# Enigmatisms/cuda-pt

Measured on AMD Instinct MI355X. Metric: Msamples/sec (whole node), 1080p modern-kitchen, higher is better.
Workload: dtype fp32; 1 GPU; model=modern-kitchen-proc, global_batch=32, seq_len=2073600, width=1920, height=1080, renderer=pt, n_prims=131444, parallelism=dp1 (sample-split, RCCL all-reduce)

## Files before the change

csrc/bind.cpp:

```cpp
#include <pybind11/pybind11.h>
#include <pybind11/numpy.h>
#include <pybind11/stl.h>
#include <algorithm>
#include <cstring>
#include <stdexcept>

#include "core/scene_view.h"
#include "core/integrator.h"
#include "cpu/bvh_build.h"
#include "hip/kernels.h"
#include "hip/lds_plan.h"

namespace py = pybind11;
using namespace hippt;

namespace hippt {
void render_cpu(const SceneView& sv, float* accum, float* var,
                int spp0, int nspp, uint32_t seed, int renderer, int n_threads,
                int y0, int y1, const uint8_t* spp_map, float* aux);
void render_lt_cpu(const SceneView& sv, float* accum, int spp0, int nspp, uint32_t seed,
                   int spec_constraint, float caustic_scaling, int n_threads);
}

namespace {

using farr = py::array_t<float, py::array::c_style | py::array::forcecast>;
using iarr = py::array_t<int32_t, py::array::c_style | py::array::forcecast>;
using uarr = py::array_t<uint32_t, py::array::c_style | py::array::forcecast>;

#define HIP_OK(expr)                                                                   \
    do {                                                                               \
        int _e = (expr);                                                               \
        if (_e != 0) throw std::runtime_error(std::string("HIP error ") +              \
                                              std::to_string(_e) + " at " #expr);      \
    } while (0)

Vec3 to_vec3(const std::vector<float>& v) { return {v[0], v[1], v[2]}; }

int super_cell_voxels() {
    static const int SUP = [] {
        const char* e = getenv("HIPPT_SUPER_N");
        int v = e ? atoi(e) : 16;
        return v < 2 ? 2 : (v > 64 ? 64 : v);
    }();
    return SUP;
}

inline void super_splat(std::vector<float>& sup, const MediumParams& m, int SUP,
                        int ix, int iy, int iz, float v) {
    int cx0 = std::max(0, (ix - 1) / SUP), cx1 = std::min(m.sx - 1, (ix + 1) / SUP);
    int cy0 = std::max(0, (iy - 1) / SUP), cy1 = std::min(m.sy - 1, (iy + 1) / SUP);
    int cz0 = std::max(0, (iz - 1) / SUP), cz1 = std::min(m.sz - 1, (iz + 1) / SUP);
    for (int cz = cz0; cz <= cz1; ++cz)
        for (int cy = cy0; cy <= cy1; ++cy)
            for (int cx = cx0; cx <= cx1; ++cx) {
                float& s = sup[(size_t(cz) * m.sy + cy) * m.sx + cx];
                s = fmaxf(s, v);
            }
}

int bvh4_tree_depth(const BVH4Node* nodes, int n) {
    if (n <= 0) return 0;
    std::vector<std::pair<int, int>> stk{{0, 1}};
    int maxd = 1;
    while (!stk.empty()) {
        auto [idx, d] = stk.back();
        stk.pop_back();
        maxd = std::max(maxd, d);
        const BVH4Node& nd = nodes[idx];
        for (int c = 0; c < 4; ++c)
            if (nd.child[c] >= 0 && !(nd.child[c] == 0 && nd.cnt[c] == 0))
                stk.push_back({nd.child[c], d + 1});
    }
    return maxd;
}

static std::vector<uint64_t> host_lds_slots(int lds_n);

std::vector<uint32_t> make_prim_shade(const uint32_t* prim_obj, size_t n_prims,
                                      const int32_t* objs, size_t n_objs) {
    std::vector<uint32_t> out(n_prims);
    int bad = -1;
    if (!build_prim_shade(prim_obj, (int)n_prims, objs, (int)n_objs, out.data(), &bad))
        throw std::runtime_error(
            "build_prim_shade: primitive " + std::to_string(bad) +
            " needs object < n_objs, 0 <= bsdf_id < " + std::to_string(SHADE_MAX_BSDFS) +
            " and emitter_id < " + std::to_string(SHADE_MAX_EMITTERS));
    return out;
}

struct SceneHolder {
    farr np_prims, np_attrs, np_nodes, np_nodes4, np_nodes8;
    uarr np_prim_obj;
    iarr np_objs;
    std::vector<BsdfParams> bsdfs;
    std::vector<EmitterParams> emitters;
    std::vector<PhaseParams> phases;
    std::vector<MediumParams> media;
    std::vector<farr> media_density, media_temp;
    std::vector<std::vector<float>> media_super;
    std::vector<std::vector<int32_t>> media_bricks;
    std::vector<int> media_nbricks;
    std::vector<farr> tex_data;
    std::vector<TexView> tex_host;
    std::vector<int> emitter_prims;
    std::vector<float> emitter_cdf;
    std::vector<uint32_t> prim_shade;
    std::vector<LightPrim> light_prims;
    bool shade_stale = true;
    std::vector<float> env_rows_h, env_cols_h;
    int env_w = 0, env_h = 0;
    std::vector<float> emitter_sel_h;
    Camera cam{};
    MaxDepthParams md{};
    int env_emitter = -1;
    int cam_medium = -1;

    bool has_dev = false;
    int device_id = 0;
    std::vector<void*> dev_bufs;
    std::vector<TexView> tex_dev;
    std::vector<MediumParams> media_dev;
    void* dev_bsdfs = nullptr;
    void* dev_emitters = nullptr;
    void* dev_media = nullptr;

    SceneView host_sv{};
    SceneView dev_sv{};
    WfState* wf = nullptr;

    ~SceneHolder() { release(); }

    void release() {
        if (wf) { wf_destroy(wf); wf = nullptr; }
        for (void* p : dev_bufs) dev_free(p);
        dev_bufs.clear();
        has_dev = false;
    }

    void set_geometry(farr prims, farr attrs, uarr prim_obj, farr nodes, farr nodes4,
                      farr nodes8) {
        if (prims.ndim() != 2 || prims.shape(1) != 12) throw std::runtime_error("prims must be (n,12)");
        if (attrs.ndim() != 2 || attrs.shape(1) != 16) throw std::runtime_error("attrs must be (n,16)");
        if (nodes.ndim() != 2 || nodes.shape(1) != 8) throw std::runtime_error("nodes must be (m,8)");
        if (nodes4.ndim() == 2 && nodes4.shape(0) > 0 && nodes4.shape(1) != 32)
            throw std::runtime_error("nodes4 must be (m,32)");
        np_prims = std::move(prims);
        np_attrs = std::move(attrs);
        np_prim_obj = std::move(prim_obj);
        shade_stale = true;
        np_nodes = std::move(nodes);
        np_nodes4 = std::move(nodes4);
        if (nodes8.ndim() == 2 && nodes8.shape(0) > 0 && nodes8.shape(1) != 64)
            throw std::runtime_error("nodes8 must be (m,64)");
        np_nodes8 = std::move(nodes8);
        bvh4_depth = np_nodes4.ndim() == 2 && np_nodes4.shape(0) > 0
            ? bvh4_tree_depth((const BVH4Node*)np_nodes4.data(), (int)np_nodes4.shape(0))
            : 0;
        nodes4q = np_nodes4.ndim() == 2 && np_nodes4.shape(0) > 0
            ? quantize_bvh4((const BVH4Node*)np_nodes4.data(), (int)np_nodes4.shape(0))
            : std::vector<BVH4NodeQ>();
        nodes4t = np_nodes4.ndim() == 2 && np_nodes4.shape(0) > 0
            ? tag_bvh4((const BVH4Node*)np_nodes4.data(), (int)np_nodes4.shape(0))
            : std::vector<BVH4NodeT>();
        const Prim* pr = (const Prim*)np_prims.data();
        const uint32_t* po = np_prim_obj.data();
        int n = (int)np_prims.shape(0);
        AABB sb;
        for (int i = 0; i < n; ++i) {
            if (po[i] & PRIM_SPHERE_BIT) {
                Vec3 c = pr[i].v0.xyz();
                float rad = pr[i].v0.w;
                sb.grow(c - Vec3(rad)); sb.grow(c + Vec3(rad));
            } else {
                Vec3 v0 = pr[i].v0.xyz();
                sb.grow(v0);
                sb.grow(v0 + pr[i].e1.xyz());
                sb.grow(v0 + pr[i].e2.xyz());
            }
        }
        Vec3 c = (sb.lo + sb.hi) * 0.5f;
        float rad = n > 0 ? (sb.hi - sb.lo).length() * 0.5f : 1.f;
        scene_bound = Vec4(c, rad);
        tri_only = 1;
        for (int i = 0; i < n; ++i)
            if (po[i] & PRIM_SPHERE_BIT) { tri_only = 0; break; }
    }

    int bvh4_depth = 0;
    Vec4 scene_bound{0.f, 0.f, 0.f, 1.f};
    int cache_nodes = 0;
    int tri_only = 0;
    std::vector<BVH4NodeQ> nodes4q;
    std::vector<BVH4NodeT> nodes4t;

    void set_cache_level(int level) {
        cache_nodes = level > 0 ? (1 << (level > 12 ? 12 : level)) : 0;
    }

    void set_objects(iarr objs) {
        if (objs.ndim() != 2 || objs.shape(1) != 8) throw std::runtime_error("objs must be (n,8)");
        np_objs = std::move(objs);
        shade_stale = true;
    }

    int add_bsdf(int type, std::vector<float> kd, std::vector<float> ks, std::vector<float> kg,
                 float ior, float extra0, float extra1, std::vector<int> tex) {
        BsdfParams b = BsdfParams::make(type);
        b.kd = Vec4(kd[0], kd[1], kd[2], kd.size() > 3 ? kd[3] : 0.f);
        b.ks = Vec4(ks[0], ks[1], ks[2], ks.size() > 3 ? ks[3] : 0.f);
        b.kg = Vec4(kg[0], kg[1], kg[2], kg.size() > 3 ? kg[3] : 0.f);
        b.ior = ior; b.extra0 = extra0; b.extra1 = extra1;
        for (size_t i = 0; i < tex.size() && i < 8; ++i) b.tex[i] = (int16_t)tex[i];
        bsdfs.push_back(b);
        return (int)bsdfs.size() - 1;
    }

// ... 722 lines not shown
            }
            if (wk0.rec.prim_idx < 0) wk0.rec.t = MAX_DIST;
            if (wk1.rec.prim_idx < 0) wk1.rec.t = MAX_DIST;
            if (!same_hit(b, wk0.rec) || !same_hit(b, wk1.rec)) { ++bad; continue; }
        }
        if (n8p) {
            HitRecord w8 = ray_intersect_bvh8_ww(n8p, pr, po, r, tmax, lds, lds_n);
            bool occ8 = occlusion_test_bvh8(n8p, pr, po, r, tmax, lds, lds_n);
            bool occ_ref = occlusion_test_bvh4(n4, pr, po, r, tmax, lds, lds_n);
            if (!same_hit(b, w8) || occ8 != occ_ref) { ++bad; continue; }
        }
        bool occ_a = occlusion_test_bvh(bn, n_nodes, pr, po, r, tmax);
        bool occ_b = occlusion_test_bvh4(n4, pr, po, r, tmax, lds, lds_n);
        if (occlusion_test_bvh4_ww(t4, pr, po, r, tmax, lds, lds_n) != occ_b) { ++bad; continue; }
        if (!same_hit(a, b) || occ_a != occ_b) ++bad;
    }
    return bad;
}

int py_bvh4q_selftest(farr prims, uarr prim_obj, farr nodes4,
                      farr ray_o, farr ray_d, float tmax, int lds_n) {
    const BVH4Node* n4 = (const BVH4Node*)nodes4.data();
    int nn = (int)nodes4.shape(0);
    std::vector<BVH4NodeQ> q = quantize_bvh4(n4, nn);
    const std::vector<BVH4NodeT> t4v = tag_bvh4(n4, nn);
    const BVH4NodeT* t4 = t4v.data();
    const Prim* pr = (const Prim*)prims.data();
    const uint32_t* po = prim_obj.data();
    std::vector<uint64_t> slots = host_lds_slots(lds_n);
    LdsSlot lds = bvh_host_slot(lds_n ? slots.data() : nullptr);
    int bad = 0;
    int nr = (int)ray_o.shape(0);
    for (int i = 0; i < nr; ++i) {
        Ray r;
        r.o = {ray_o.at(i, 0), ray_o.at(i, 1), ray_o.at(i, 2)};
        r.d = {ray_d.at(i, 0), ray_d.at(i, 1), ray_d.at(i, 2)};
        HitRecord a = ray_intersect_bvh4_ww(t4, pr, po, r, tmax, lds, lds_n);
        HitRecord b = ray_intersect_bvh4q_ww(q.data(), pr, po, r, tmax, lds, lds_n);
        if (!same_hit(a, b)) { ++bad; continue; }
        bool oa = occlusion_test_bvh4_ww(t4, pr, po, r, tmax, lds, lds_n);
        bool ob = occlusion_test_bvh4q_ww(q.data(), pr, po, r, tmax, lds, lds_n);
        if (oa != ob) ++bad;
    }
    return bad;
}

uarr py_bvh4_tag(farr nodes4) {
    if (nodes4.ndim() != 2 || nodes4.shape(1) != 32) throw std::runtime_error("nodes4 must be (m,32)");
    const std::vector<BVH4NodeT> t4 =
        tag_bvh4((const BVH4Node*)nodes4.data(), (int)nodes4.shape(0));
    uarr out({(py::ssize_t)t4.size(), (py::ssize_t)32});
    std::memcpy(out.mutable_data(), t4.data(), t4.size() * sizeof(BVH4NodeT));
    return out;
}

int py_bvh4_visit_selftest(farr nodes4, farr ray_o, farr ray_d, float tmax) {
    if (nodes4.ndim() != 2 || nodes4.shape(1) != 32) throw std::runtime_error("nodes4 must be (m,32)");
    const BVH4Node* n4 = (const BVH4Node*)nodes4.data();
    const int nn = (int)nodes4.shape(0);
    const std::vector<BVH4NodeT> t4 = tag_bvh4(n4, nn);
    const LdsSlot no_lds = nullptr;
    int bad = 0;
    const int nr = (int)ray_o.shape(0);
    for (int i = 0; i < nr; ++i) {
        Ray r;
        r.o = {ray_o.at(i, 0), ray_o.at(i, 1), ray_o.at(i, 2)};
        r.d = {ray_d.at(i, 0), ray_d.at(i, 1), ray_d.at(i, 2)};
        const Vec3 inv_d = safe_rcp_dir(r.d);
        const Vec3 o_div = r.o * inv_d;
        for (int j = 0; j < nn; ++j) {
            uint64_t sa[4] = {0, 0, 0, 0}, sb[4] = {0, 0, 0, 0};
            int spa = 0, spb = 0;
            uint32_t na, nb;
            {
                const BVH4Node nd = n4[j];
                BVH_VISIT_ORDERED(BVH4Node, na, nd, inv_d, o_div, tmax, sa, spa, no_lds, 0)
            }
            {
                const BVH4NodeT nd = t4[j];
                BVH_VISIT_TAGGED4(nb, nd, inv_d, o_div, tmax, sb, spb, no_lds, 0)
            }
            if (na != nb || spa != spb || std::memcmp(sa, sb, sizeof(sa)) != 0) ++bad;
        }
    }
    return bad;
}

int py_bvh4_any_visit_selftest(farr nodes4, farr ray_o, farr ray_d, float tmax) {
    if (nodes4.ndim() != 2 || nodes4.shape(1) != 32) throw std::runtime_error("nodes4 must be (m,32)");
    const BVH4Node* n4 = (const BVH4Node*)nodes4.data();
    const int nn = (int)nodes4.shape(0);
    const std::vector<BVH4NodeT> t4 = tag_bvh4(n4, nn);
    const LdsSlot no_lds = nullptr;
    auto collect = [](uint32_t next, const uint64_t* st, int sp, uint32_t* out, int& n) {
        n = 0;
        if (next != BVH4_NONE_W) out[n++] = next;
        for (int k = 0; k < sp; ++k) {
            if (st[k] >> 32) return false;
            const uint32_t w = (uint32_t)st[k];
            if (w == BVH4_NONE_W || w == BVH4_ANY_MISS_W) return false;
            out[n++] = w;
        }
        std::sort(out, out + n);
        return std::adjacent_find(out, out + n) == out + n;
    };
    int bad = 0;
// ... 114 lines not shown
        .def("add_bsdf", &SceneHolder::add_bsdf)
        .def("update_bsdf", &SceneHolder::update_bsdf)
        .def("add_emitter", &SceneHolder::add_emitter)
        .def("update_emitter", &SceneHolder::update_emitter)
        .def("set_emitter_prims", &SceneHolder::set_emitter_prims)
        .def("set_env_cdf", &SceneHolder::set_env_cdf)
        .def("set_emitter_sel", &SceneHolder::set_emitter_sel)
        .def("add_phase", &SceneHolder::add_phase)
        .def("add_medium", &SceneHolder::add_medium)
        .def("add_medium_sparse", &SceneHolder::add_medium_sparse)
        .def("media_info", &SceneHolder::media_info)
        .def("medium_super", &SceneHolder::medium_super)
        .def("update_medium", &SceneHolder::update_medium)
        .def("add_texture", &SceneHolder::add_texture)
        .def("set_camera", &SceneHolder::set_camera)
        .def("set_depths", &SceneHolder::set_depths,
             py::arg("max_depth"), py::arg("max_diffuse"), py::arg("max_specular"),
             py::arg("max_transmit"), py::arg("max_volume"), py::arg("min_time"),
             py::arg("max_time"), py::arg("use_tof"), py::arg("radiance_clamp") = 0.f)
        .def("set_cache_level", &SceneHolder::set_cache_level)
        .def_readwrite("cam_medium", &SceneHolder::cam_medium)
        .def_readwrite("env_emitter", &SceneHolder::env_emitter)
        .def("finalize", &SceneHolder::finalize)
        .def("upload", &SceneHolder::upload)
        .def("release", &SceneHolder::release)
        .def("render_host", &SceneHolder::render_host,
             py::arg("accum"), py::arg("var"), py::arg("spp0"), py::arg("nspp"),
             py::arg("seed"), py::arg("renderer"), py::arg("spec_constraint"),
             py::arg("caustic_scaling"), py::arg("n_threads"),
             py::arg("y0") = 0, py::arg("y1") = 0, py::arg("spp_map") = py::none(),
             py::arg("aux") = py::none())
        .def("render_device", &SceneHolder::render_device,
             py::arg("accum_ptr"), py::arg("var_ptr"), py::arg("spp0"), py::arg("nspp"),
             py::arg("seed"), py::arg("renderer"), py::arg("spec_constraint"),
             py::arg("caustic_scaling"), py::arg("stream"),
             py::arg("y0") = 0, py::arg("y1") = 0, py::arg("spp_map_ptr") = 0,
             py::arg("aux_ptr") = 0)
        .def("trace_rays", &SceneHolder::trace_rays, py::arg("o"), py::arg("d"),
             py::arg("tmax"), py::arg("device"), py::arg("lds_n") = -1,
             py::arg("n_cached") = -1)
        .def("shade_probe", &SceneHolder::shade_probe_py, py::arg("prim_idx"),
             py::arg("device"))
        .def("tables", &SceneHolder::tables)
        .def("info", &SceneHolder::info);

    m.def("build_bvh", &py_build_bvh, py::arg("prims"), py::arg("prim_obj"),
          py::arg("max_leaf") = 4, py::arg("overlap_w") = 0.f,
          py::arg("use_sbvh") = false, py::arg("ref_unsplit") = true,
          py::arg("trav_cost") = 0.f);
    m.def("collapse_bvh4", &py_collapse_bvh4, py::arg("nodes"));
    m.def("collapse_bvh8", &py_collapse_bvh8, py::arg("nodes"));
    m.def("bvh4_hit", &py_bvh4_hit);
    m.def("bvh4_tag", &py_bvh4_tag, py::arg("nodes4"));
    m.def("bvh4_visit_selftest", &py_bvh4_visit_selftest, py::arg("nodes4"),
          py::arg("ray_o"), py::arg("ray_d"), py::arg("tmax"));
    m.def("bvh4_any_visit_selftest", &py_bvh4_any_visit_selftest, py::arg("nodes4"),
          py::arg("ray_o"), py::arg("ray_d"), py::arg("tmax"));
    m.def("build_prim_shade", [](uarr prim_obj, iarr objs) {
        if (objs.ndim() != 2 || objs.shape(1) != 8) throw std::runtime_error("objs must be (n,8)");
        std::vector<uint32_t> w = make_prim_shade(prim_obj.data(), (size_t)prim_obj.size(),
                                                  objs.data(), (size_t)objs.shape(0));
        uarr out((py::ssize_t)w.size());
        if (!w.empty()) std::memcpy(out.mutable_data(), w.data(), w.size() * 4);
        return out;
    }, py::arg("prim_obj"), py::arg("objs"));
    m.def("build_light_prims", [](farr prims, farr attrs, uarr prim_obj, iarr emitter_prims) {
        if (prims.ndim() != 2 || prims.shape(1) != 12) throw std::runtime_error("prims must be (n,12)");
        if (attrs.ndim() != 2 || attrs.shape(1) != 16) throw std::runtime_error("attrs must be (n,16)");
        const py::ssize_t n_prims = prims.shape(0);
        if (attrs.shape(0) != n_prims || prim_obj.size() != n_prims)
            throw std::runtime_error("prims, attrs and prim_obj must have one row per primitive");
        const py::ssize_t n = emitter_prims.size();
        for (py::ssize_t k = 0; k < n; ++k)
            if (emitter_prims.data()[k] < 0 || emitter_prims.data()[k] >= n_prims)
                throw std::runtime_error("emitter_prims entry outside the primitive array");
        uarr out({n, (py::ssize_t)32});
        build_light_prims((const Prim*)prims.data(), (const PrimAttr*)attrs.data(),
                          prim_obj.data(), emitter_prims.data(), (size_t)n,
                          (LightPrim*)out.mutable_data());
        return out;
    }, py::arg("prims"), py::arg("attrs"), py::arg("prim_obj"), py::arg("emitter_prims"));
    m.def("bsdf_check", &py_bsdf_check);
    m.def("env_check", &py_env_check);
    m.def("bvh4q_selftest", &py_bvh4q_selftest,
          py::arg("prims"), py::arg("prim_obj"), py::arg("nodes4"),
          py::arg("ray_o"), py::arg("ray_d"), py::arg("tmax"), py::arg("lds_n") = 0);
    m.def("bvh4_selftest", &py_bvh4_selftest,
          py::arg("prims"), py::arg("prim_obj"), py::arg("nodes"), py::arg("nodes4"),
          py::arg("ray_o"), py::arg("ray_d"), py::arg("tmax"),
          py::arg("nodes8") = farr(), py::arg("lds_n") = 0);

    m.def("wf_sort_probe", [](uarr status, uarr gather, int mode) {
        if (status.ndim() != 1 || gather.ndim() != 1)
            throw std::runtime_error("wf_sort_probe: status (n,), gather (m,) or empty");
        const int n = (int)status.shape(0), m = (int)gather.shape(0);
        uarr out(n);
        int live = -1;
        HIP_OK(wf_sort_probe(status.data(), n, gather.data(), m, mode,
                             out.mutable_data(), &live));
        return py::make_tuple(out, live);
    }, py::arg("status"), py::arg("gather"), py::arg("mode"));
    m.def("lds_plan", [](int occ, bool stack_in_lds, bool scratch_drops_cache, int n_nodes4,
                         int node_bytes, int cache_req, int lds_req) {
        if (n_nodes4 < 0 || node_bytes <= 0) throw std::runtime_error("lds_plan: bad sizes");
        const LdsPlan p = lds_plan(occ, stack_in_lds, scratch_drops_cache, n_nodes4,
                                   node_bytes, cache_req, lds_req);
        return py::make_tuple(p.lds_n, p.n_cached, p.shmem);
    }, py::arg("occ"), py::arg("stack_in_lds"), py::arg("scratch_drops_cache"),
       py::arg("n_nodes4"), py::arg("node_bytes"), py::arg("cache_req"),
       py::arg("lds_req") = -1);
    m.def("dev_synchronize", [] { HIP_OK(dev_synchronize()); });
    m.def("dev_set_device", [](int d) { HIP_OK(dev_set_device(d)); });

    m.def("struct_sizes", [] {
        py::dict d;
        d["BVHNode"] = (int)sizeof(BVHNode);
        d["Prim"] = (int)sizeof(Prim);
        d["PrimAttr"] = (int)sizeof(PrimAttr);
        d["ObjInfo"] = (int)sizeof(ObjInfo);
        d["BsdfParams"] = (int)sizeof(BsdfParams);
        d["EmitterParams"] = (int)sizeof(EmitterParams);
        d["MediumParams"] = (int)sizeof(MediumParams);
        d["PhaseParams"] = (int)sizeof(PhaseParams);
        d["TexView"] = (int)sizeof(TexView);
        d["Camera"] = (int)sizeof(Camera);
        d["SceneView"] = (int)sizeof(SceneView);
        return d;
    });

    m.attr("R_MEGAKERNEL_PT") = (int)R_MEGAKERNEL_PT;
    m.attr("R_WAVEFRONT_PT") = (int)R_WAVEFRONT_PT;
    m.attr("R_VOLUME_PT") = (int)R_VOLUME_PT;
    m.attr("R_LIGHT_TRACE") = (int)R_LIGHT_TRACE;
    m.attr("R_DEPTH") = (int)R_DEPTH;
    m.attr("R_BVH_COST") = (int)R_BVH_COST;
    m.attr("R_MEGAKERNEL_PT_DYN") = (int)R_MEGAKERNEL_PT_DYN;
    m.attr("WAVE_SIZE") = 64;
}
```

csrc/core/bvh4.h:

```cpp
#pragma once
#include <stdexcept>
#include "bvh.h"

namespace hippt {

template <int W>
struct alignas(16) BVHWideNode {
    static constexpr int WIDTH = W;
    static constexpr bool EMPTY_BEFORE_BOX = false;
    static constexpr bool TAGGED = false;
    float lo_x[W], lo_y[W], lo_z[W];
    float hi_x[W], hi_y[W], hi_z[W];
    int32_t child[W];
    int32_t cnt[W];
};
using BVH4Node = BVHWideNode<4>;
static_assert(sizeof(BVH4Node) == 128, "BVH4Node must be 128 bytes");

struct alignas(16) BVH4NodeT {
    static constexpr int WIDTH = 4;
    static constexpr bool EMPTY_BEFORE_BOX = false;
    static constexpr bool TAGGED = true;
    float lo_x[4], lo_y[4], lo_z[4];
    float hi_x[4], hi_y[4], hi_z[4];
    uint32_t child[4];
    uint32_t pad[4];
};
static_assert(sizeof(BVH4NodeT) == 128, "BVH4NodeT must be 128 bytes");

struct alignas(16) BVH4NodeQ {
    static constexpr int WIDTH = 4;
    static constexpr bool EMPTY_BEFORE_BOX = true;
    static constexpr bool TAGGED = true;
    float ox, oy, oz;
    uint8_t ex, ey, ez;
    uint8_t pad;
    uint8_t qlo[4][3];
    uint8_t qhi[4][3];
    uint32_t child[4];
};
static_assert(sizeof(BVH4NodeQ) == 64, "BVH4NodeQ must be 64 bytes");

constexpr int BVH4_STACK = 64;

constexpr uint32_t BVH4_NONE_W = 0x7fffffffu;
HD uint32_t bvh4_filled_word(int ch, int pc) {
    return ch < 0 ? (0x80000000u | ((uint32_t)pc << 27) | (uint32_t)(~ch)) : (uint32_t)ch;
}
HD uint32_t bvh4_child_word(int ch, int pc) {
    if (ch < 0 && pc == 0) return BVH4_NONE_W;
    return bvh4_filled_word(ch, pc);
}
HD bool bvh4_is_leaf(uint32_t w) { return w >= 0x80000000u; }
HD bool bvh4_not_leaf(uint32_t w) { return w < 0x80000000u; }
// ... 245 lines not shown
    }
#define BVH_VISIT_ANY4(next, nd, inv_d, o_div, tmax, stack, sp, lds_slot, lds_n) \
    BVH_ANY_WORD4(w0_, nd, 0, inv_d, o_div, tmax)                         \
    BVH_ANY_WORD4(w1_, nd, 1, inv_d, o_div, tmax)                         \
    BVH_ANY_WORD4(w2_, nd, 2, inv_d, o_div, tmax)                         \
    BVH_ANY_WORD4(w3_, nd, 3, inv_d, o_div, tmax)                         \
    BVH_ANY_MINMAX(w0_, w1_)                                              \
    BVH_ANY_MINMAX(w2_, w3_)                                              \
    BVH_ANY_MINMAX(w0_, w2_)                                              \
    BVH_ANY_MINMAX(w1_, w3_)                                              \
    BVH_ANY_MINMAX(w1_, w2_)                                              \
    BVH_PUSH_ANY4(w3_, stack, sp, lds_slot, lds_n)                        \
    BVH_PUSH_ANY4(w2_, stack, sp, lds_slot, lds_n)                        \
    BVH_PUSH_ANY4(w1_, stack, sp, lds_slot, lds_n)                        \
    next = w0_ == BVH4_ANY_MISS_W ? BVH4_NONE_W : w0_;

HD Prim bvh_load_prim(const Prim* prims, const uint32_t* prim_obj, int pid,
                      bool tri_only, bool& sph) {
    uint32_t obj = 0;
    if (!tri_only) obj = prim_obj[pid];
    const Prim p = prims[pid];
#if HIPPT_ON_DEVICE
    asm volatile("" :: "v"(obj), "v"(p.v0.x), "v"(p.v0.y), "v"(p.v0.z), "v"(p.v0.w),
                       "v"(p.e1.x), "v"(p.e1.y), "v"(p.e1.z), "v"(p.e1.w),
                       "v"(p.e2.x), "v"(p.e2.y), "v"(p.e2.z), "v"(p.e2.w));
#endif
    sph = (obj & PRIM_SPHERE_BIT) != 0;
    return p;
}
HD void bvh4_leaf_hit(const Prim* prims, const uint32_t* prim_obj,
                      const Ray& ray, int base, int cnt, HitRecord& rec,
                      bool tri_only = false) {
    for (int k = 0; k < cnt; ++k) {
        int pid = base + k;
        bool sph;
        const Prim p = bvh_load_prim(prims, prim_obj, pid, tri_only, sph);
        float u, v;
        float t = intersect_prim(p, sph, ray, u, v);
        if (t > EPSILON && t < rec.t) {
            rec.t = t; rec.u = u; rec.v = v; rec.prim_idx = pid;
        }
    }
}
#define BVH_LEAF_ANY_RETURN(prims, prim_obj, ray, base, cnt, tmax, tri_only)  \
    for (int k_ = 0; k_ < (cnt); ++k_) {                                      \
        int pid_ = (base) + k_;                                               \
        bool sph_;                                                            \
        const Prim p_ = bvh_load_prim(prims, prim_obj, pid_, tri_only, sph_); \
        float u_, v_;                                                         \
        float t_ = intersect_prim(p_, sph_, ray, u_, v_);                     \
        if (t_ > EPSILON && t_ < (tmax)) return true;                         \
    }

template <class Node>
HD HitRecord bvh_closest_ww(const Node* nodes, const Prim* prims,
                            const uint32_t* prim_obj, const Ray& ray, float tmax,
                            LdsSlot lds_slot, int lds_n, const Node* top_cache,
                            int n_cached, bool tri_only) {
    HitRecord rec;
    rec.t = tmax;
    const Vec3 inv_d = safe_rcp_dir(ray.d);
    const Vec3 o_div = ray.o * inv_d;
    uint64_t stack[BVH4_STACK];
    int sp = 0;
    uint32_t cur = 0;
    for (;;) {
        while (bvh4_is_node(cur)) {
            const Node* nsrc = (int)cur < n_cached ? top_cache : nodes;
            const Node nd = nsrc[cur];
            uint32_t next;
            BVH_VISIT(Node, next, nd, inv_d, o_div, rec.t, stack, sp, lds_slot, lds_n)
            if (next != BVH4_NONE_W) { cur = next; continue; }
            BVH_POP_CLOSER(cur, stack, sp, lds_slot, lds_n, rec.t, break, break)
        }
        if (cur == BVH4_NONE_W) break;
        while (bvh4_is_leaf(cur)) {
            bvh4_leaf_hit(prims, prim_obj, ray, bvh4_leaf_base(cur),
                          bvh4_leaf_count(cur), rec, tri_only);
            BVH_POP_CLOSER(cur, stack, sp, lds_slot, lds_n, rec.t, break, break)
        }
        if (cur == BVH4_NONE_W) break;
    }
    if (rec.prim_idx < 0) rec.t = MAX_DIST;
    return rec;
}
template <class Node>
HD bool bvh_any_ww(const Node* nodes, const Prim* prims, const uint32_t* prim_obj,
                   const Ray& ray, float tmax, LdsSlot lds_slot, int lds_n,
                   const Node* top_cache, int n_cached, bool tri_only) {
    const Vec3 inv_d = safe_rcp_dir(ray.d);
    const Vec3 o_div = ray.o * inv_d;
    uint64_t stack[BVH4_STACK];
    int sp = 0;
    uint32_t cur = 0;
    for (;;) {
        while (bvh4_is_node(cur)) {
            const Node* nsrc = (int)cur < n_cached ? top_cache : nodes;
            const Node nd = nsrc[cur];
            uint32_t next = BVH4_NONE_W;
            if constexpr (BVH4_ANY_STRAIGHT && Node::WIDTH == 4 && Node::TAGGED) {
                BVH_VISIT_ANY4(next, nd, inv_d, o_div, tmax, stack, sp, lds_slot, lds_n)
            } else {
                BVH_VISIT_ANY_EACH(Node, next, nd, inv_d, o_div, tmax, stack, sp, lds_slot, lds_n)
            }
            if (next != BVH4_NONE_W) { cur = next; continue; }
            BVH_POP_WORD(cur, stack, sp, lds_slot, lds_n, break)
        }
        if (cur == BVH4_NONE_W) return false;
        while (bvh4_is_leaf(cur)) {
            const int base = bvh4_leaf_base(cur), pc = bvh4_leaf_count(cur);
            BVH_LEAF_ANY_RETURN(prims, prim_obj, ray, base, pc, tmax, tri_only)
            BVH_POP_WORD(cur, stack, sp, lds_slot, lds_n, break)
        }
        if (cur == BVH4_NONE_W) return false;
    }
}

HD HitRecord ray_intersect_bvh4_ww(const BVH4NodeT* nodes,
                                   const Prim* prims, const uint32_t* prim_obj,
                                   const Ray& ray, float tmax,
                                   LdsSlot lds_slot = nullptr, int lds_n = 0,
                                   const BVH4NodeT* top_cache = nullptr,
                                   int n_cached = 0, bool tri_only = false) {
    return bvh_closest_ww(nodes, prims, prim_obj, ray, tmax, lds_slot, lds_n,
                          top_cache, n_cached, tri_only);
}
HD bool occlusion_test_bvh4_ww(const BVH4NodeT* nodes,
                               const Prim* prims, const uint32_t* prim_obj,
                               const Ray& ray, float tmax,
                               LdsSlot lds_slot = nullptr, int lds_n = 0,
                               const BVH4NodeT* top_cache = nullptr,
                               int n_cached = 0, bool tri_only = false) {
    return bvh_any_ww(nodes, prims, prim_obj, ray, tmax, lds_slot, lds_n,
                      top_cache, n_cached, tri_only);
}
HD HitRecord ray_intersect_bvh4q_ww(const BVH4NodeQ* nodes,
                                    const Prim* prims, const uint32_t* prim_obj,
                                    const Ray& ray, float tmax,
                                    LdsSlot lds_slot = nullptr, int lds_n = 0,
                                    const BVH4NodeQ* top_cache = nullptr,
                                    int n_cached = 0) {
    return bvh_closest_ww(nodes, prims, prim_obj, ray, tmax, lds_slot, lds_n,
                          top_cache, n_cached, false);
}
HD bool occlusion_test_bvh4q_ww(const BVH4NodeQ* nodes,
                                const Prim* prims, const uint32_t* prim_obj,
                                const Ray& ray, float tmax,
                                LdsSlot lds_slot = nullptr, int lds_n = 0,
                                const BVH4NodeQ* top_cache = nullptr,
                                int n_cached = 0) {
    return bvh_any_ww(nodes, prims, prim_obj, ray, tmax, lds_slot, lds_n,
// ... 106 lines not shown
}

struct Bvh4Walk {
    HitRecord rec;
    uint32_t cur;
    int sp;
    Vec3 inv_d, o_div;
    Ray ray;
    uint64_t stack[BVH4_STACK / 2];
};

HD void bvh4_walk_init(Bvh4Walk& w, const Ray& ray, float tmax) {
    w.rec = HitRecord();
    w.rec.t = tmax;
    w.cur = 0;
    w.sp = 0;
    w.inv_d = safe_rcp_dir(ray.d);
    w.o_div = ray.o * w.inv_d;
    w.ray = ray;
}

HD bool bvh4_walk_step(Bvh4Walk& w, const BVH4NodeT* nodes, const Prim* prims,
                       const uint32_t* prim_obj, LdsSlot lds_slot, int lds_n) {
    if (w.cur == BVH4_NONE_W) return false;
    if (bvh4_not_leaf(w.cur)) {
        const BVH4NodeT nd = nodes[w.cur];
        uint32_t next;
        BVH_VISIT_TAGGED4(next, nd, w.inv_d, w.o_div, w.rec.t,
                          w.stack, w.sp, lds_slot, lds_n)
        if (next != BVH4_NONE_W) { w.cur = next; return true; }
    } else {
        bvh4_leaf_hit(prims, prim_obj, w.ray, bvh4_leaf_base(w.cur),
                      bvh4_leaf_count(w.cur), w.rec);
    }
    BVH_POP_CLOSER(w.cur, w.stack, w.sp, lds_slot, lds_n, w.rec.t, return false, return true)
}

inline std::vector<BVH4NodeT> tag_bvh4(const BVH4Node* nodes, int n) {
    std::vector<BVH4NodeT> out((size_t)(n > 0 ? n : 0));
    for (int i = 0; i < n; ++i) {
        const BVH4Node& s = nodes[i];
        BVH4NodeT& t = out[i];
        std::memcpy(t.lo_x, s.lo_x, 6 * 4 * sizeof(float));
        for (int c = 0; c < 4; ++c) {
            if (s.child[c] < 0 && (int64_t)(~s.child[c]) + s.cnt[c] > BVH4_MAX_PRIMS)
                throw std::runtime_error("tag_bvh4: leaf beyond BVH4_MAX_PRIMS prims");
            t.child[c] = bvh4_child_word(s.child[c], s.cnt[c]);
            t.pad[c] = 0;
        }
    }
    return out;
}

inline std::vector<BVH4NodeQ> quantize_bvh4(const BVH4Node* nodes, int n) {
    std::vector<BVH4NodeQ> out((size_t)n);
    for (int i = 0; i < n; ++i) {
        const BVH4Node& s = nodes[i];
        BVH4NodeQ& q = out[i];
        float lo[3] = {3e38f, 3e38f, 3e38f}, hi[3] = {-3e38f, -3e38f, -3e38f};
        for (int c = 0; c < 4; ++c) {
            if (s.child[c] == 0 && s.cnt[c] == 0) continue;
            lo[0] = fminf(lo[0], s.lo_x[c]); hi[0] = fmaxf(hi[0], s.hi_x[c]);
            lo[1] = fminf(lo[1], s.lo_y[c]); hi[1] = fmaxf(hi[1], s.hi_y[c]);
            lo[2] = fminf(lo[2], s.lo_z[c]); hi[2] = fmaxf(hi[2], s.hi_z[c]);
        }
        if (lo[0] > hi[0]) { lo[0] = lo[1] = lo[2] = 0.f; hi[0] = hi[1] = hi[2] = 0.f; }
        q.ox = lo[0]; q.oy = lo[1]; q.oz = lo[2];
        uint8_t* eptr = &q.ex;
        for (int a = 0; a < 3; ++a) {
            float ext = fmaxf(hi[a] - lo[a], 0.f);
            int e = 127;
            if (ext > 0.f) {
                float need = ext / 255.f;
                int ee;
                frexpf(need, &ee);
                e = 127 + ee;
                if (e < 1) e = 1;
                if (e > 254) e = 254;
            }
            eptr[a] = (uint8_t)e;
        }
        q.pad = 0;
        const float sxyz[3] = {bvh4q_scale(q.ex), bvh4q_scale(q.ey), bvh4q_scale(q.ez)};
        for (int c = 0; c < 4; ++c) {
            if (s.child[c] == 0 && s.cnt[c] == 0) {
                q.child[c] = BVH4_NONE_W;
                for (int a = 0; a < 3; ++a) { q.qlo[c][a] = 255; q.qhi[c][a] = 0; }
                continue;
            }
            const float clo[3] = {s.lo_x[c], s.lo_y[c], s.lo_z[c]};
            const float chi[3] = {s.hi_x[c], s.hi_y[c], s.hi_z[c]};
            for (int a = 0; a < 3; ++a) {
                float inv_s = 1.f / sxyz[a];
                float fl = floorf((clo[a] - (&q.ox)[a]) * inv_s);
                float fh = ceilf((chi[a] - (&q.ox)[a]) * inv_s);
                q.qlo[c][a] = (uint8_t)clampv((int)fl, 0, 255);
                q.qhi[c][a] = (uint8_t)clampv((int)fh, 0, 255);
            }
            q.child[c] = bvh4_child_word(s.child[c], s.cnt[c]);
        }
    }
    return out;
}

}
```

csrc/hip/pt_kernels.hip:

```cpp
#include <hip/hip_runtime.h>
#include "kernels.h"
#include "trav_lds.h"
#include <climits>
#include "../core/integrator.h"
#include "../core/integrator_vol.h"
#include "../core/light_tracer.h"

namespace hippt {

__device__ inline int xcd_swizzle(int flat, int n_tiles) {
    int xcd = flat & 7, local = flat >> 3;
    int per = n_tiles >> 3, rem = n_tiles & 7;
    return xcd * per + (xcd < rem ? xcd : rem) + local;
}

template <int RENDERER, int MINW, bool BRICKS = false>
__global__ __launch_bounds__(256)
__attribute__((amdgpu_waves_per_eu(MINW, MINW)))
void k_render(SceneView sv, float* __restrict__ accum, float* __restrict__ var,
              int spp0, int nspp, uint32_t seed, int swiz, int lds_n, int n_cached, int y_off, int y_end,
              const uint8_t* __restrict__ spp_map, float* __restrict__ aux) {
    extern __shared__ uint64_t s_stk[];
    TravCtx tc = trav_lds_ctx(sv, s_stk, threadIdx.y * 16 + threadIdx.x, lds_n, n_cached);
    int tile = blockIdx.y * gridDim.x + blockIdx.x;
// ... 78 lines not shown
            Sampler sp(uint32_t(pix), uint32_t(spp0 + s) * SEED_SCALER + seed);
            Ray ray = sv.cam.gen_ray(px, py, sp, spp0 + s);
            Vec3 L = trace_path(sv, ray, sp, tc);
            Lsum += L;
            float lum = (L.x + L.y + L.z) * (1.f / 3.f);
            lum_s += lum;
            lum_s2 = fmaf(lum, lum, lum_s2);
        }
        float* a = accum + pix * 4;
        a[0] += Lsum.x; a[1] += Lsum.y; a[2] += Lsum.z; a[3] += (float)nspp;
        if (var) { var[pix * 2 + 0] += lum_s; var[pix * 2 + 1] += lum_s2; }
    }
}

__global__ __launch_bounds__(256)
__attribute__((amdgpu_waves_per_eu(6, 6)))
void k_render_lt(SceneView sv, float* __restrict__ accum,
                 long long n_paths, int spp0, int nspp, uint32_t seed,
                 int spec_constraint, float caustic_scaling, int lds_n) {
    extern __shared__ uint64_t s_stk[];
    TravCtx tc{(LdsSlot)&s_stk[threadIdx.x], lds_n};
    const long long stride = (long long)gridDim.x * blockDim.x;
    for (long long i = (long long)blockIdx.x * blockDim.x + threadIdx.x; i < n_paths; i += stride) {
        Sampler sp(uint32_t(i & 0xffffffff), uint32_t(spp0) * SEED_SCALER + seed + uint32_t(i >> 32));
        trace_light_path_impl(sv, sp, [&](int pix, Vec3 v) {
            atomicAdd(accum + pix * 4 + 0, v.x);
            atomicAdd(accum + pix * 4 + 1, v.y);
            atomicAdd(accum + pix * 4 + 2, v.z);
        }, tc, spec_constraint, caustic_scaling);
    }
}

__global__ void k_add_count(float* __restrict__ accum, size_t npix, float cnt) {
    size_t i = (size_t)blockIdx.x * blockDim.x + threadIdx.x;
    if (i < npix) accum[i * 4 + 3] += cnt;
}

int launch_render(const SceneView& sv, float* accum, float* var,
                  int spp0, int nspp, uint32_t seed, int renderer,
                  int spec_constraint, float caustic_scaling, void* stream,
                  int y0, int y1, const uint8_t* spp_map, float* aux) {
    hipStream_t st = (hipStream_t)stream;
    static const int swiz_v = env_int("HIPPT_SWIZZLE", 0);
    const int swiz = renderer == R_DEPTH || renderer == R_BVH_COST ? 0 : swiz_v;
    constexpr int OCC_PT = 4, OCC_VPT = 4, OCC_REST = 4, OCC_UNSET = INT_MIN;
    static const int occ_env = env_int("HIPPT_OCC", OCC_UNSET);
    const bool is_rest = renderer == R_LIGHT_TRACE || renderer == R_DEPTH ||
                         renderer == R_BVH_COST || renderer == R_MEGAKERNEL_PT_DYN;
    const int occ_v = occ_env != OCC_UNSET ? occ_env
                    : renderer == R_VOLUME_PT ? OCC_VPT
                    : is_rest ? OCC_REST : OCC_PT;
    static const bool stack_in_lds = !env_is("HIPPT_STACK", "scratch");
    const LdsPlan plan = lds_plan(occ_v, stack_in_lds, false, sv.n_nodes4,
                                  (int)sizeof(TravNode), top_cache_request(sv));
    const int lds_n = plan.lds_n, n_cached = plan.n_cached;
    const uint32_t shmem = plan.shmem;
    const int w = sv.cam.w, h = sv.cam.h;
    if (y1 <= 0 || y1 > h) y1 = h;
    if (y0 < 0) y0 = 0;
    dim3 block(16, 16);
    dim3 grid((w + 15) / 16, (y1 - y0 + 15) / 16);
    void (*k)(SceneView, float*, float*, int, int, uint32_t, int, int, int, int, int,
              const uint8_t*, float*) = nullptr;
    switch (renderer) {
    case R_LIGHT_TRACE: {
        long long n_paths = (long long)w * h * nspp;
        int nblk = 256 * 8 * 4;
        hipLaunchKernelGGL(k_render_lt, dim3(nblk), dim3(256), shmem, st,
                           sv, accum, n_paths, spp0, nspp, seed, spec_constraint, caustic_scaling, lds_n);
        size_t npix = (size_t)w * h;
        hipLaunchKernelGGL(k_add_count, dim3((npix + 255) / 256), dim3(256), 0, st,
                           accum, npix, (float)nspp);
        break;
    }
    case R_VOLUME_PT:
        if (sv.media_bricks) k = occ_v == 4 ? k_render<R_VOLUME_PT, 4, true> : k_render<R_VOLUME_PT, 6, true>;
        else k = occ_v == 4 ? k_render<R_VOLUME_PT, 4> : k_render<R_VOLUME_PT, 6>;
        break;
    case R_DEPTH: k = k_render<R_DEPTH, 6>; break;
    case R_BVH_COST: k = k_render<R_BVH_COST, 6>; break;
    case R_MEGAKERNEL_PT_DYN: {
        static struct Counters {
            uint32_t* p[64] = {};
            ~Counters() { for (uint32_t* q : p) if (q) (void)hipFree(q); }
        } counters;
        int dev = 0;
        (void)hipGetDevice(&dev);
        uint32_t*& counter = counters.p[dev & 63];
        if (!counter) {
            if (hipMalloc((void**)&counter, 4) != hipSuccess) return (int)hipGetLastError();
        }
        (void)hipMemsetAsync(counter, 0, 4, st);
        int tiles_x = (w + 15) / 16, tiles_y = (h + 15) / 16;
        hipLaunchKernelGGL((k_render_persistent<R_MEGAKERNEL_PT, 6>), dim3(256 * 4), block, shmem, st,
                           sv, accum, var, spp0, nspp, seed, counter, tiles_x,
                           tiles_x * tiles_y, lds_n);
        break;
    }
    default:
        if (occ_v <= 3) k = k_render<R_MEGAKERNEL_PT, 3>;
        else if (occ_v == 4) k = k_render<R_MEGAKERNEL_PT, 4>;
        else if (occ_v == 5) k = k_render<R_MEGAKERNEL_PT, 5>;
        else if (occ_v >= 8) k = k_render<R_MEGAKERNEL_PT, 8>;
        else k = k_render<R_MEGAKERNEL_PT, 6>;
        break;
    }
    if (k) hipLaunchKernelGGL(k, grid, block, shmem, st, sv, accum, var, spp0, nspp, seed,
// ... 17 lines not shown
```

csrc/hip/trav_lds.h:

```cpp
#pragma once
#include <hip/hip_runtime.h>
#include <cstdlib>
#include <cstring>
#include "lds_plan.h"
#include "../core/scene_view.h"

namespace hippt {

inline int env_int(const char* name, int dflt) {
    const char* e = getenv(name);
    return e ? atoi(e) : dflt;
}
inline bool env_is(const char* name, const char* value) {
    const char* e = getenv(name);
    return e && strcmp(e, value) == 0;
}

inline int top_cache_request(const SceneView& sv, int probe = -1) {
    static const int cache_env = env_int("HIPPT_TOPCACHE", -1);
    return probe >= 0 ? probe : cache_env >= 0 ? cache_env
         : sv.cache_nodes > 0 ? sv.cache_nodes : 64;
}

__device__ __forceinline__ TravCtx trav_lds_ctx(const SceneView& sv, uint64_t* s_stk,
                                                int tid, int lds_n, int n_cached) {
    constexpr int NW = (int)(sizeof(TravNode) / 8);
    TravNode* s_cache = (TravNode*)s_stk;
    uint64_t* s_base = s_stk + (size_t)n_cached * NW;
    for (int i = tid; i < n_cached * NW; i += LDS_BLOCK)
        ((uint64_t*)s_cache)[i] = ((const uint64_t*)trav_nodes(sv))[i];
    if (n_cached > 0) __syncthreads();
    return TravCtx{(LdsSlot)&s_base[tid], lds_n, s_cache, n_cached};
}

}
```

csrc/hip/wf_kernels.hip:

```cpp
#include <hip/hip_runtime.h>
#include "kernels.h"
#include "trav_lds.h"
#include "../core/integrator.h"

namespace hippt {

constexpr int WF_BLOCK = 256;
constexpr int SORT_BLOCK = 256;
constexpr int SORT_ITEMS = 16;
constexpr uint32_t DEAD = 0x80u;

struct WfState {
    int w = 0, h = 0, n = 0;
    int nb_sort = 0;
    float4* ray_o = nullptr;
    float4* ray_d = nullptr;
    float4* thp = nullptr;
    float4* L = nullptr;
    float4* hit = nullptr;
    float4* prevn = nullptr;
    unsigned long long* rng = nullptr;
    uint32_t* status = nullptr;
    uint32_t* order = nullptr;
    uint32_t* order2 = nullptr;
// ... 482 lines not shown
    (void)nspp_done;
}

template <typename T>
static int wf_alloc(T** p, size_t count) { return (int)hipMalloc((void**)p, count * sizeof(T)); }

WfState* wf_create(int width, int height) {
    if ((long long)width * height > WF_MAX_PIXELS) return nullptr;
    WfState* s = new WfState();
    s->w = width; s->h = height; s->n = width * height;
    s->nb_sort = (s->n + SORT_BLOCK * SORT_ITEMS - 1) / (SORT_BLOCK * SORT_ITEMS);
    int e = 0;
    e |= wf_alloc(&s->ray_o, s->n);
    e |= wf_alloc(&s->ray_d, s->n);
    e |= wf_alloc(&s->thp, s->n);
    e |= wf_alloc(&s->L, s->n);
    e |= wf_alloc(&s->hit, s->n);
    e |= wf_alloc(&s->prevn, s->n);
    e |= wf_alloc(&s->rng, s->n);
    e |= wf_alloc(&s->status, s->n);
    e |= wf_alloc(&s->order, s->n);
    e |= wf_alloc(&s->order2, s->n);
    e |= wf_alloc(&s->hist, (size_t)s->nb_sort * 256);
    e |= wf_alloc(&s->live_dev, 1);
    e |= wf_alloc(&s->sh_od, s->n);
    e |= wf_alloc(&s->sh_dir, s->n);
    e |= wf_alloc(&s->sh_val, s->n);
    e |= wf_alloc(&s->sh_cnt, 1);
    e |= (int)hipHostMalloc((void**)&s->live_host, sizeof(int));
    if (e) { wf_destroy(s); return nullptr; }
    return s;
}

void wf_destroy(WfState* s) {
    if (!s) return;
    (void)hipFree(s->ray_o); (void)hipFree(s->ray_d); (void)hipFree(s->thp); (void)hipFree(s->L);
    (void)hipFree(s->hit); (void)hipFree(s->prevn); (void)hipFree(s->rng);
    (void)hipFree(s->status); (void)hipFree(s->order); (void)hipFree(s->order2);
    (void)hipFree(s->hist);
    (void)hipFree(s->live_dev);
    (void)hipFree(s->sh_od); (void)hipFree(s->sh_dir); (void)hipFree(s->sh_val); (void)hipFree(s->sh_cnt);
    if (s->live_host) (void)hipHostFree(s->live_host);
    delete s;
}

static int wf_occ() {
    static const int occ = env_int("HIPPT_WF_OCC", 4);
    return occ < 3 ? 3 : (occ > 6 ? 6 : occ);
}
#define WF_BY_OCC(k) (wf_occ() == 3 ? k<3> : wf_occ() == 4 ? k<4> : wf_occ() == 5 ? k<5> : k<6>)

static LdsPlan wf_lds_plan(const SceneView& sv, int lds_req = -1, int cache_in = -1) {
    static const bool stack_in_lds = !env_is("HIPPT_WF_STACK", "scratch");
    return lds_plan(wf_occ(), stack_in_lds, true, sv.n_nodes4, (int)sizeof(TravNode),
                    top_cache_request(sv, cache_in), lds_req);
}

int launch_render_wavefront(WfState* st, const SceneView& sv, float* accum, float* var,
                            int spp0, int nspp, uint32_t seed, int sort_mode, void* stream) {
    if (sort_mode < 0 || sort_mode > 1) sort_mode = 0;
    static const int env_mode = env_is("HIPPT_WF_SORT", "compact") ? 1 : -1;
    if (env_mode >= 0) sort_mode = env_mode;
    hipStream_t hs = (hipStream_t)stream;
    const int n = st->n;
    dim3 blk(WF_BLOCK);
    dim3 grd_n((n + WF_BLOCK - 1) / WF_BLOCK);
    static const auto f_raygen = WF_BY_OCC(k_wf_raygen);
    static const auto f_primary = WF_BY_OCC(k_wf_primary);
    static const auto f_trace = WF_BY_OCC(k_wf_trace);
    static const auto f_tail = WF_BY_OCC(k_wf_tail);
    static const auto f_step = WF_BY_OCC(k_wf_step);
    static const auto f_shadow = WF_BY_OCC(k_wf_shadow);
    static const int prim_fuse = env_int("HIPPT_WF_PRIMARY_FUSE", 1);
    static const int wf_fuse = env_int("HIPPT_WF_FUSE", 1);
    static const int span_env = env_int("HIPPT_WF_SPAN", 8);
    static const int wf_span = span_env < 1 ? 1 : (span_env > 16 ? 16 : span_env);
    const LdsPlan plan = wf_lds_plan(sv);
    const int n_cached = plan.n_cached;
    const int lds_n = plan.lds_n;
    const uint32_t shmem = plan.shmem;
    static int wf_dual = env_int("HIPPT_WF_DUAL", 0);
    if (wf_dual && 3 * sv.bvh4_depth > BVH4_STACK / 2 + lds_n / 2) wf_dual = 0;
    static const int tail_thresh = env_int("HIPPT_WF_TAIL", 1500 * 1024);
    static const int wf_log = env_int("HIPPT_WF_LOG", 0);
    for (int s = 0; s < nspp; ++s) {
        int bounce0;
        const int n_stage = sv.md.max_depth + 1;
        if (prim_fuse && wf_fuse) {
            int cnt = wf_span < n_stage ? wf_span : n_stage;
            hipLaunchKernelGGL(f_primary, grd_n, blk, shmem, hs, sv, *st, spp0 + s,
                               seed, cnt - 1, cnt < n_stage ? 1 : 0, lds_n, n_cached);
            bounce0 = cnt;
        } else {
            hipLaunchKernelGGL(f_raygen, grd_n, blk, shmem, hs, sv, *st, spp0 + s, seed,
                               lds_n, n_cached);
            bounce0 = 0;
        }
        const uint32_t* gather = nullptr;
        int prev_live = n;
        uint32_t* order_cur = st->order;
        uint32_t* order_prev = st->order2;
        for (int bounce = bounce0; bounce < n_stage; bounce += (wf_fuse ? wf_span : 1)) {
            const int scan_n = prev_live;
            wf_sort_launch(st->status, gather, scan_n, st->hist, st->live_dev,
                           order_cur, sort_mode, hs);
            (void)hipMemcpyAsync(st->live_host, st->live_dev, sizeof(int),
                                 hipMemcpyDeviceToHost, hs);
// ... 159 lines not shown
```

setup.py:

```python
import os
import subprocess
import sys
import sysconfig
from pathlib import Path

ROOT = Path(__file__).resolve().parent
HIPCC = os.environ.get("HIPCC", "/opt/rocm/bin/hipcc")
ARCH = os.environ.get("HIPPT_ARCH", "gfx950")

SOURCES = [
    "csrc/bind.cpp",
    "csrc/cpu/bvh_build.cpp",
    "csrc/cpu/sbvh_build.cpp",
    "csrc/cpu/cpu_render.cpp",
    "csrc/hip/pt_kernels.hip",
    "csrc/hip/wf_kernels.hip",
]


def pybind11_includes():
    import pybind11
    return [pybind11.get_include()]


def compile_flags():
    cflags = [
        "-O3", "-std=c++17", "-fPIC", f"--offload-arch={ARCH}",
        "-ffast-math", "-fno-finite-math-only",
        "-Wno-unused-result",
    ]
    if os.environ.get("HIPPT_QBVH"):
        cflags.append("-DHIPPT_QBVH")
    ldflags = []
    if os.environ.get("HIPPT_DEBUG"):
        cflags = [f for f in cflags if f not in ("-O3", "-ffast-math")]
        cflags += ["-O1", "-g"]
    if os.environ.get("HIPPT_ASAN"):
        cflags += ["-fsanitize=address", "-shared-libasan"]
        ldflags += ["-fsanitize=address", "-shared-libasan"]
    return cflags, ldflags


def build(verbose=True):
    py_inc = sysconfig.get_paths()["include"]
    ext = sysconfig.get_config_var("EXT_SUFFIX") or ".so"
    out = ROOT / "hippt" / f"_C{ext}"
    objdir = ROOT / "build" / "obj"
    objdir.mkdir(parents=True, exist_ok=True)
    incs = [f"-I{py_inc}"] + [f"-I{p}" for p in pybind11_includes()]
    cflags, ldflags = compile_flags()
    stamp = objdir / ".flags"
    flags_now = " ".join(cflags)
    if not stamp.exists() or stamp.read_text() != flags_now:
        for o in objdir.glob("*.o"):
            o.unlink()
        stamp.write_text(flags_now)
    objs = []
    procs = []
    for src in SOURCES:
        sp = ROOT / src
        obj = objdir / (sp.stem + ".o")
        objs.append(str(obj))
        if obj.exists() and obj.stat().st_mtime > max(
            sp.stat().st_mtime,
            max((h.stat().st_mtime for h in (ROOT / "csrc").rglob("*.h")), default=0),
        ):
            continue
        cmd = [HIPCC, "-c", str(sp), "-o", str(obj)] + cflags + incs
        if src.endswith(".hip"):
            cmd += ["-x", "hip"]
        if verbose:
            print("[hippt build]", " ".join(cmd), flush=True)
        procs.append(subprocess.Popen(cmd))
    for p in procs:
        if p.wait() != 0:
            raise SystemExit(f"hipcc failed ({p.args[2]})")
    link = [HIPCC, "-shared", "-fPIC", f"--offload-arch={ARCH}", "-o", str(out)] + objs + ldflags
    if verbose:
        print("[hippt build]", " ".join(link), flush=True)
    subprocess.check_call(link)
    return out


if __name__ == "__main__":
    if len(sys.argv) > 1 and sys.argv[1] == "clean":
# ... 5 lines not shown
```

Baseline: 307.6 Msamples/s.

## Reorder BVH4 nodes so the largest-area top nodes fill the LDS cache

Renumbers BVH4 nodes at scene load: the first 512 slots are chosen best-first by child surface area (level or DFS order via env), and the rest keep their original order. This lets the LDS top-node cache, which holds the lowest-indexed nodes, hold the nodes most rays visit. It also adds an optional padded LDS stride for cached nodes, meant to reduce bank conflicts, but the default stride of 128 adds no padding. The cost is extra host preprocessing and lost DFS locality for the reordered top nodes.

New measurement: 321.2 Msamples/s (median of 6 runs). 4.4% higher.

```diff
diff --git a/csrc/bind.cpp b/csrc/bind.cpp
--- a/csrc/bind.cpp
+++ b/csrc/bind.cpp
@@ -2,8 +2,10 @@
 #include <pybind11/numpy.h>
 #include <pybind11/stl.h>
 #include <algorithm>
+#include <cstdlib>
 #include <cstring>
 #include <stdexcept>
+#include <string>
 
 #include "core/scene_view.h"
 #include "core/integrator.h"
@@ -87,6 +89,15 @@
             " needs object < n_objs, 0 <= bsdf_id < " + std::to_string(SHADE_MAX_BSDFS) +
             " and emitter_id < " + std::to_string(SHADE_MAX_EMITTERS));
     return out;
+}
+
+static BVH4TopOrder top_order_from(const char* name) {
+    if (!name || !*name) return BVH4_TOP_ORDER_DEFAULT;
+    const std::string s(name);
+    if (s == "area") return TOP_AREA;
+    if (s == "level") return TOP_LEVEL;
+    if (s == "dfs") return TOP_DFS;
+    throw std::runtime_error("top order must be area, level or dfs, not '" + s + "'");
 }
 
 struct SceneHolder {
@@ -157,12 +168,16 @@
         bvh4_depth = np_nodes4.ndim() == 2 && np_nodes4.shape(0) > 0
             ? bvh4_tree_depth((const BVH4Node*)np_nodes4.data(), (int)np_nodes4.shape(0))
             : 0;
-        nodes4q = np_nodes4.ndim() == 2 && np_nodes4.shape(0) > 0
-            ? quantize_bvh4((const BVH4Node*)np_nodes4.data(), (int)np_nodes4.shape(0))
-            : std::vector<BVH4NodeQ>();
-        nodes4t = np_nodes4.ndim() == 2 && np_nodes4.shape(0) > 0
-            ? tag_bvh4((const BVH4Node*)np_nodes4.data(), (int)np_nodes4.shape(0))
-            : std::vector<BVH4NodeT>();
+        nodes4q.clear();
+        nodes4t.clear();
+        if (np_nodes4.ndim() == 2 && np_nodes4.shape(0) > 0) {
+            std::vector<int32_t> perm;
+            const std::vector<BVH4Node> top = bvh4_top_first(
+                (const BVH4Node*)np_nodes4.data(), (int)np_nodes4.shape(0), BVH4_TOP_ORDERED,
+                top_order_from(getenv("HIPPT_TOP_ORDER")), perm);
+            nodes4q = quantize_bvh4(top.data(), (int)top.size());
+            nodes4t = tag_bvh4(top.data(), (int)top.size());
+        }
         const Prim* pr = (const Prim*)np_prims.data();
         const uint32_t* po = np_prim_obj.data();
         int n = (int)np_prims.shape(0);
@@ -991,6 +1006,19 @@
     uarr out({(py::ssize_t)t4.size(), (py::ssize_t)32});
     std::memcpy(out.mutable_data(), t4.data(), t4.size() * sizeof(BVH4NodeT));
     return out;
+}
+
+py::tuple py_bvh4_top_first(farr nodes4, int n_top, const std::string& order) {
+    if (nodes4.ndim() != 2 || nodes4.shape(1) != 32) throw std::runtime_error("nodes4 must be (m,32)");
+    std::vector<int32_t> perm;
+    const std::vector<BVH4Node> top = bvh4_top_first(
+        (const BVH4Node*)nodes4.data(), (int)nodes4.shape(0), n_top,
+        top_order_from(order.c_str()), perm);
+    farr out({(py::ssize_t)top.size(), (py::ssize_t)32});
+    std::memcpy(out.mutable_data(), top.data(), top.size() * sizeof(BVH4Node));
+    iarr p((py::ssize_t)perm.size());
+    std::memcpy(p.mutable_data(), perm.data(), perm.size() * sizeof(int32_t));
+    return py::make_tuple(out, p);
 }
 
 int py_bvh4_visit_selftest(farr nodes4, farr ray_o, farr ray_d, float tmax) {
@@ -1211,6 +1239,8 @@
     m.def("collapse_bvh8", &py_collapse_bvh8, py::arg("nodes"));
     m.def("bvh4_hit", &py_bvh4_hit);
     m.def("bvh4_tag", &py_bvh4_tag, py::arg("nodes4"));
+    m.def("bvh4_top_first", &py_bvh4_top_first, py::arg("nodes4"),
+          py::arg("n_top") = BVH4_TOP_ORDERED, py::arg("order") = "");
     m.def("bvh4_visit_selftest", &py_bvh4_visit_selftest, py::arg("nodes4"),
           py::arg("ray_o"), py::arg("ray_d"), py::arg("tmax"));
     m.def("bvh4_any_visit_selftest", &py_bvh4_any_visit_selftest, py::arg("nodes4"),
@@ -1295,4 +1325,6 @@
     m.attr("R_BVH_COST") = (int)R_BVH_COST;
     m.attr("R_MEGAKERNEL_PT_DYN") = (int)R_MEGAKERNEL_PT_DYN;
     m.attr("WAVE_SIZE") = 64;
-}
+    m.attr("BVH4_TOP_ORDERED") = BVH4_TOP_ORDERED;
+    m.attr("TRAV_CACHE_STRIDE") = bvh_cache_stride<TravNode>();
+}
diff --git a/csrc/core/bvh4.h b/csrc/core/bvh4.h
--- a/csrc/core/bvh4.h
+++ b/csrc/core/bvh4.h
@@ -1,5 +1,7 @@
 #pragma once
+#include <queue>
 #include <stdexcept>
+#include <vector>
 #include "bvh.h"
 
 namespace hippt {
@@ -351,6 +353,28 @@
         if (t_ > EPSILON && t_ < (tmax)) return true;                         \
     }
 
+#ifndef HIPPT_CACHE_STRIDE
+#define HIPPT_CACHE_STRIDE 128
+#endif
+constexpr int TRAV_CACHE_STRIDE = HIPPT_CACHE_STRIDE;
+static_assert(TRAV_CACHE_STRIDE >= 128 && TRAV_CACHE_STRIDE % 16 == 0,
+              "cached nodes are read with 16-byte loads");
+template <class Node>
+constexpr int bvh_cache_stride() { return (int)sizeof(Node) + (TRAV_CACHE_STRIDE - 128); }
+template <class Node>
+HD const Node* bvh_node_at(const Node* nodes, const Node* top_cache, int n_cached,
+                           uint32_t cur) {
+    constexpr uint32_t PAD16 = (uint32_t)(bvh_cache_stride<Node>() - (int)sizeof(Node)) / 16u;
+    const bool cached = (int)cur < n_cached;
+    const Node* nsrc = cached ? top_cache : nodes;
+    if constexpr (PAD16 == 0) {
+        return nsrc + cur;
+    } else {
+        const uint32_t units = cur * (uint32_t)(sizeof(Node) / 16) + (cached ? cur * PAD16 : 0u);
+        return (const Node*)((const char*)nsrc + (size_t)units * 16);
+    }
+}
+
 template <class Node>
 HD HitRecord bvh_closest_ww(const Node* nodes, const Prim* prims,
                             const uint32_t* prim_obj, const Ray& ray, float tmax,
@@ -365,8 +389,7 @@
     uint32_t cur = 0;
     for (;;) {
         while (bvh4_is_node(cur)) {
-            const Node* nsrc = (int)cur < n_cached ? top_cache : nodes;
-            const Node nd = nsrc[cur];
+            const Node nd = *bvh_node_at(nodes, top_cache, n_cached, cur);
             uint32_t next;
             BVH_VISIT(Node, next, nd, inv_d, o_div, rec.t, stack, sp, lds_slot, lds_n)
             if (next != BVH4_NONE_W) { cur = next; continue; }
@@ -394,8 +417,7 @@
     uint32_t cur = 0;
     for (;;) {
         while (bvh4_is_node(cur)) {
-            const Node* nsrc = (int)cur < n_cached ? top_cache : nodes;
-            const Node nd = nsrc[cur];
+            const Node nd = *bvh_node_at(nodes, top_cache, n_cached, cur);
             uint32_t next = BVH4_NONE_W;
             if constexpr (BVH4_ANY_STRAIGHT && Node::WIDTH == 4 && Node::TAGGED) {
                 BVH_VISIT_ANY4(next, nd, inv_d, o_div, tmax, stack, sp, lds_slot, lds_n)
@@ -608,6 +630,68 @@
     return out;
 }
 
+constexpr int BVH4_TOP_ORDERED = 512;
+enum BVH4TopOrder { TOP_DFS = 0, TOP_LEVEL = 1, TOP_AREA = 2 };
+constexpr BVH4TopOrder BVH4_TOP_ORDER_DEFAULT = TOP_AREA;
+inline std::vector<BVH4Node> bvh4_top_first(const BVH4Node* nodes, int n, int n_top,
+                                            BVH4TopOrder order, std::vector<int32_t>& perm) {
+    if (n < 0) n = 0;
+    perm.resize((size_t)n);
+    for (int i = 0; i < n; ++i) perm[i] = i;
+    std::vector<BVH4Node> out(nodes, nodes + n);
+    const int k_top = n_top < n ? n_top : n;
+    if (order == TOP_DFS || k_top <= 1) return out;
+    for (int i = 0; i < n; ++i)
+        for (int c = 0; c < 4; ++c)
+            if (nodes[i].child[c] >= n)
+                throw std::runtime_error("bvh4_top_first: child index beyond the node array");
+    struct Open { double prio; int node; };
+    struct Later {
+        bool operator()(const Open& a, const Open& b) const {
+            return a.prio < b.prio || (a.prio == b.prio && a.node > b.node);
+        }
+    };
+    std::priority_queue<Open, std::vector<Open>, Later> open;
+    std::vector<int> depth((size_t)n, 0);
+    std::vector<char> placed((size_t)n, 0);
+    std::vector<int> src;
+    src.reserve((size_t)n);
+    auto place = [&](int i) {
+        placed[i] = 1;
+        src.push_back(i);
+        const BVH4Node& s = nodes[i];
+        for (int c = 0; c < 4; ++c) {
+            const int ch = s.child[c];
+            if (ch < 0 || placed[ch]) continue;
+            depth[ch] = depth[i] + 1;
+            double prio = -(double)depth[ch];
+            if (order == TOP_AREA) {
+                const double dx = (double)s.hi_x[c] - (double)s.lo_x[c];
+                const double dy = (double)s.hi_y[c] - (double)s.lo_y[c];
+                const double dz = (double)s.hi_z[c] - (double)s.lo_z[c];
+                prio = 2.0 * (dx * dy + dy * dz + dz * dx);
+                if (!(prio >= 0.0)) prio = 0.0;
+            }
+            open.push({prio, ch});
+        }
+    };
+    place(0);
+    while ((int)src.size() < k_top && !open.empty()) {
+        const int i = open.top().node;
+        open.pop();
+        if (!placed[i]) place(i);
+    }
+    for (int i = 0; i < n; ++i)
+        if (!placed[i]) src.push_back(i);
+    for (int k = 0; k < n; ++k) perm[src[k]] = k;
+    for (int k = 0; k < n; ++k) {
+        out[k] = nodes[src[k]];
+        for (int c = 0; c < 4; ++c)
+            if (out[k].child[c] >= 0) out[k].child[c] = perm[out[k].child[c]];
+    }
+    return out;
+}
+
 inline std::vector<BVH4NodeQ> quantize_bvh4(const BVH4Node* nodes, int n) {
     std::vector<BVH4NodeQ> out((size_t)n);
     for (int i = 0; i < n; ++i) {
diff --git a/csrc/hip/pt_kernels.hip b/csrc/hip/pt_kernels.hip
--- a/csrc/hip/pt_kernels.hip
+++ b/csrc/hip/pt_kernels.hip
@@ -154,7 +154,7 @@
                     : is_rest ? OCC_REST : OCC_PT;
     static const bool stack_in_lds = !env_is("HIPPT_STACK", "scratch");
     const LdsPlan plan = lds_plan(occ_v, stack_in_lds, false, sv.n_nodes4,
-                                  (int)sizeof(TravNode), top_cache_request(sv));
+                                  TRAV_CACHE_NODE_BYTES, top_cache_request(sv));
     const int lds_n = plan.lds_n, n_cached = plan.n_cached;
     const uint32_t shmem = plan.shmem;
     const int w = sv.cam.w, h = sv.cam.h;
diff --git a/csrc/hip/trav_lds.h b/csrc/hip/trav_lds.h
--- a/csrc/hip/trav_lds.h
+++ b/csrc/hip/trav_lds.h
@@ -22,13 +22,17 @@
          : sv.cache_nodes > 0 ? sv.cache_nodes : 64;
 }
 
+constexpr int TRAV_CACHE_NODE_BYTES = bvh_cache_stride<TravNode>();
+
 __device__ __forceinline__ TravCtx trav_lds_ctx(const SceneView& sv, uint64_t* s_stk,
                                                 int tid, int lds_n, int n_cached) {
     constexpr int NW = (int)(sizeof(TravNode) / 8);
+    constexpr int SW = TRAV_CACHE_NODE_BYTES / 8;
+    static_assert((NW & (NW - 1)) == 0 && TRAV_CACHE_NODE_BYTES % 8 == 0, "word split");
     TravNode* s_cache = (TravNode*)s_stk;
-    uint64_t* s_base = s_stk + (size_t)n_cached * NW;
+    uint64_t* s_base = s_stk + (size_t)n_cached * SW;
     for (int i = tid; i < n_cached * NW; i += LDS_BLOCK)
-        ((uint64_t*)s_cache)[i] = ((const uint64_t*)trav_nodes(sv))[i];
+        s_stk[(i / NW) * SW + (i % NW)] = ((const uint64_t*)trav_nodes(sv))[i];
     if (n_cached > 0) __syncthreads();
     return TravCtx{(LdsSlot)&s_base[tid], lds_n, s_cache, n_cached};
 }
diff --git a/csrc/hip/wf_kernels.hip b/csrc/hip/wf_kernels.hip
--- a/csrc/hip/wf_kernels.hip
+++ b/csrc/hip/wf_kernels.hip
@@ -558,7 +558,7 @@
 
 static LdsPlan wf_lds_plan(const SceneView& sv, int lds_req = -1, int cache_in = -1) {
     static const bool stack_in_lds = !env_is("HIPPT_WF_STACK", "scratch");
-    return lds_plan(wf_occ(), stack_in_lds, true, sv.n_nodes4, (int)sizeof(TravNode),
+    return lds_plan(wf_occ(), stack_in_lds, true, sv.n_nodes4, TRAV_CACHE_NODE_BYTES,
                     top_cache_request(sv, cache_in), lds_req);
 }
 
diff --git a/setup.py b/setup.py
--- a/setup.py
+++ b/setup.py
@@ -31,6 +31,8 @@
     ]
     if os.environ.get("HIPPT_QBVH"):
         cflags.append("-DHIPPT_QBVH")
+    if os.environ.get("HIPPT_CACHE_STRIDE"):
+        cflags.append("-DHIPPT_CACHE_STRIDE=" + str(int(os.environ["HIPPT_CACHE_STRIDE"])))
     ldflags = []
     if os.environ.get("HIPPT_DEBUG"):
         cflags = [f for f in cflags if f not in ("-O3", "-ffast-math")]
```
